# amcerbu/huygens

Hardware: AMD Instinct MI355X
Metric: band-samples/s (bands x frames/s) for 4096-band Filterbank (higher is better)
Workload: dtype f64; 1 GPU; C2 Filterbank<double>(order 2, 4096 bands), resonant band-pass f_i=0.5(i+1)SR/4096 R=0.999, boost 1 + open, k_p=0.1 k_g=1; samples_per_gpu=480000, bands=4096, bands_per_gpu=4096

## Files before the change

huygens_amd/_lib.py:

```python
from __future__ import annotations

import ctypes as C
import os
import re

_HERE = os.path.dirname(os.path.abspath(__file__))
LIB_PATH = os.environ.get("HZ_LIB_PATH") or os.path.join(_HERE, "lib", "libhuygens_hip.so")
HEADER_PATH = os.path.join(os.path.dirname(_HERE), "include", "huygens_hip.h")

HZ_OK = 0
HZ_E_INVALID = -1
HZ_E_RANGE = -2
HZ_E_HIP = -3
HZ_E_NODEV = -4
HZ_E_ALLOC = -5
HZ_E_UNSUPPORTED = -6
HZ_E_STATE = -7

HZ_FB_PATH_AUTO = 0
HZ_FB_PATH_GENERAL = 1
HZ_FB_PATH_LTI = 2
HZ_FB_PATH_RESPONSE = 3
HZ_FB_PATH_STREAM = 4

# ... 67 lines not shown
    "hz_fb_profile_read": (I, [VP, PD, PD, PD, C.POINTER(L)]),
    "hz_fb_set_target_groups": (I, [VP, I]),
    "hz_fb_set_path": (I, [VP, I]),
    "hz_fb_last_path": (I, [VP, C.POINTER(I)]),
    "hz_fb_tune_lti": (I, [VP, I, I, I]),
    "hz_fb_lti_plan": (I, [VP, C.POINTER(C.c_long), C.POINTER(C.c_long), C.POINTER(C.c_int)]),
    "hz_fb_lti_last_chunk": (I, [VP, C.POINTER(C.c_int)]),
    "hz_fb_set_response": (I, [VP, I]),
    "hz_fb_tune_response": (I, [VP, L, L]),
    "hz_fb_tune_response_engine": (I, [VP, I]),
    "hz_fb_sample_many": (I, [C.POINTER(VP), I, PD, I, D, PD]),
    "hz_fb_response_engine": (I, [VP, C.POINTER(I), C.POINTER(I)]),
    "hz_fb_tune_modal": (I, [VP, I]),
    "hz_fb_modal_info": (I, [VP, C.POINTER(I), C.POINTER(I), C.POINTER(I), C.POINTER(I)]),
    "hz_fb_response_info": (I, [VP, C.POINTER(L), C.POINTER(L), C.POINTER(I), C.POINTER(L)]),
    "hz_fb_get_response": (I, [VP, PD, L]),
    "hz_fb_set_bank_response": (I, [VP, PD, L]),
    "hz_fb_set_time_shard": (I, [VP, I, I]),
    "hz_fb_set_time_shard_fill": (I, [VP, I]),
    "hz_fb_time_shard_info": (I, [VP, C.POINTER(I), C.POINTER(L), C.POINTER(L), L]),
    "hz_fb_stationary_ready": (I, [VP, L, C.POINTER(I)]),
    "hz_fb_arm_time_shard": (I, [VP, I]),
    "hz_fb_tune_stream": (I, [VP, I]),
    "hz_fb_setter_seq": (I, [VP, C.POINTER(C.c_longlong)]),
    "hz_dly_sample": (I, [VP, VP, VP, I]),
    "hz_gran_sample": (I, [VP, D, PD]),
    "hz_rt_info": (I, [I, C.POINTER(C.c_longlong), C.POINTER(C.c_longlong), C.POINTER(I)]),
    "hz_add_lookahead_info": (I, [VP, C.POINTER(L), C.POINTER(L), C.POINTER(L)]),
    "hz_fb_stream_info": (I, [VP, C.POINTER(I), C.POINTER(L), C.POINTER(L), C.POINTER(I)]),
    "hz_osc_create": (I, [I, D, I, C.POINTER(VP)]),
# ... 202 lines not shown
```

huygens_amd/csrc/hz_fb_impl.h:

```cpp
#pragma once

#include <algorithm>
#include <atomic>
#include <chrono>
#include <cmath>
#include <cstring>
#include <mutex>
#include <optional>
#include <vector>

#include "hz_common.h"
#include "hz_fb_events.h"
#include "hz_mix.h"
#include "hz_mixplan.h"

namespace hz_fbi {

constexpr int kMaxOrder = 4;
constexpr int kLtiGeomChunk128 = 3;
constexpr int kStreamBlock = 1024;
constexpr size_t kLdsCeiling = 160 * 1024;

enum { MODE_MIX = 0, MODE_SEGEND = 1, MODE_STATE = 2 };

// ... 75 lines not shown
    std::vector<double> pg_host;
    long mirror_clock = 0;
    std::vector<long> mirror_at;
    bool converged = false;
    std::vector<hz::Event> sync_ev;
    hz::DevBuf<double> d_xhist_red;
    hz::PinBuf<double> tv_row;
    hz::Event tv_ev;
    bool tv_pending = false;
    int tv_kind = 0;
    double tv_param = 0;
    struct Resp {
        int mode = HZ_FB_RESP_EAGER;
        long K = -2;
        bool h_valid = false;
        long run = 0;
        bool implicit = false;
        long calls = 0;
        long min_call = 0;
        long bands_per_sample = -1;
        std::vector<double> h_over;
        bool over_valid = false;
        int shard_rank = 0, shard_world = 1;
        bool shard_zero = true;
        bool armed = false;
        hz::DevBuf<double> d_hist[2];
        int hcur = 0;
        hz::DevBuf<double> d_h;
        hz::DevBuf<double> d_hpart;
        hz::DevBuf<double> d_coef;
// ... 211 lines not shown
```

huygens_amd/csrc/hz_fb_mac.h:

```cpp
#pragma once

#include <hip/hip_runtime.h>

#include <algorithm>
#include <type_traits>

#include "hz_lds.h"

namespace hz_mac {

constexpr int kH = 2048;
constexpr int kMacR = 8;

enum StorePolicy { kStPlain = 0, kStThrough = 1 };
#ifndef HZ_ST_Y
#define HZ_ST_Y kStThrough
#endif
constexpr int kStY = HZ_ST_Y;
typedef unsigned int hz_u32x4 __attribute__((ext_vector_type(4)));
template <int POL>
struct Store16 {
    double2* base;
    __amdgpu_buffer_rsrc_t rs;
    __device__ __forceinline__ Store16(double2* b, unsigned bytes) : base(b) {
// ... 129 lines not shown
    const int b0 = (blockIdx.x / (kH / kMacBins)) * kMacBlk;
    HZ_DIAG_AT(1, 0);
    const long row_lo = (long)b0 + Q - QP;
    double2 hv[kHL], zv[kZL];
    auto hload = [&](auto k_) {
        constexpr int k = decltype(k_)::value;
        const double2 v = H[(long)(sl + 4 * k) * kH + q];
        hv[k] = make_double2(v.x, v.y);
    };
    auto zload = [&](auto k_) {
        constexpr int k = decltype(k_)::value;
        const int r = sl + 4 * k;
        const long row = row_lo + r;
        zv[k] = 4 * k + 3 < kZr || r < kZr ? Z[(row > 0 ? row : 0) * kH + q] : make_double2(0.0, 0.0);
    };
    constexpr int OS = S < QP ? S : (QP > 8 ? 8 : QP);
    static_for<0, QP / OS>([&](auto s_) {
        constexpr int s = decltype(s_)::value;
        static_for<s * OS / 4, (s + 1) * OS / 4>(hload);
        static_for_down<mac_zhi(QP, kZL, s, OS), mac_zlo(QP, s, OS)>(zload);
    });
    HZ_DIAG_VMCNT(kHL - OS / 4 + (QP - OS) / 4);
    HZ_DIAG_AT(1, 1);
    double ar[BPW], ai[BPW], zr[BPW], zi[BPW];
    static_for<0, NS>([&](auto s_) {
        constexpr int s = decltype(s_)::value;
        if constexpr (s == NS - 1) {
            HZ_DIAG_VMCNT(0);
            HZ_DIAG_AT(1, 2);
        }
        static_for<s * S / 4, (s + 1) * S / 4>([&](auto k_) {
// ... 43 lines not shown
            for (int r = 0; r < BPW; ++r) asm volatile("" : "+v"(ar[r]), "+v"(ai[r]));
            __builtin_amdgcn_sched_barrier(0);
        }
    });
    HZ_DIAG_AT(1, 3);
    const int nb = min(B - b0, kMacBlk);
    const Store16<kStY> yst(Y + (long)b0 * kH + q0, (unsigned)sizeof(double2) * ((nb - 1) * kH + kMacBins));
#pragma unroll
    for (int r = 0; r < BPW; ++r) {
        const int lb = BPW * sl + r;
        if (lb < nb) yst(lb * kH + lq, make_double2(ar[r], ai[r]));
    }
    HZ_DIAG_AT(1, 4);
}

constexpr int kMacChunk = 24;
constexpr int kMaccBins = 16;
constexpr size_t kMaccLdsBytes = sizeof(double2) * kMaccBins * (kMacChunk + (256 / kMaccBins) * kMacBpw + kMacChunk - 1);
__global__ __launch_bounds__(256) void resp_mac_kernel_ldsc(const double2* __restrict__ H, const double2* __restrict__ Z,
                                                            double2* __restrict__ Y, int Q, int B, int nch, int cps,
                                                            long ystride) {
    constexpr int BINS = kMaccBins, BPW = kMacBpw;
    constexpr int QP = kMacChunk, SL = 256 / BINS, kMacBlk = SL * BPW, kZr = kMacBlk + QP - 1;
    constexpr int kHL = (QP + SL - 1) / SL, kZL = (kZr + SL - 1) / SL;
    extern __shared__ double2 mac_lds[];
    double2(*hs)[BINS] = (double2(*)[BINS])mac_lds;
    double2(*zs)[BINS] = (double2(*)[BINS])(mac_lds + QP * BINS);
    const int t = threadIdx.x, lq = t & (BINS - 1), sl = t / BINS;
    const int q0 = (blockIdx.x % (kH / BINS)) * BINS, q = q0 + lq;
    const int b0 = (blockIdx.x / (kH / BINS)) * kMacBlk;
    double2 hv[kHL], zv[kZL];
// ... 68 lines not shown
template <int QP, int S = mac_stage<QP>()>
int launch_mac_lds_qp(int device, int B, const double2* H, const double2* Z, double2* Y, int Q, hipStream_t s) {
    if (int r = hz::allow_lds(device, (const void*)resp_mac_kernel_lds<QP, S>, mac_lds_bytes<QP>())) return r;
    hipLaunchKernelGGL((resp_mac_kernel_lds<QP, S>), dim3(mac_lds_grid(B)), dim3(256), (mac_lds_bytes<QP>()), s, H, Z, Y, Q, B);
    return HZ_OK;
}
inline int launch_mac_lds(int device, int Qp, int B, const double2* H, const double2* Z, double2* Y, int Q, hipStream_t s) {
    if (Qp > kMacChunk) {
        constexpr int blk = (256 / kMaccBins) * kMacBpw;
        const int ns = macc_splits(Qp), nch = Qp / kMacChunk, cps = (nch + ns - 1) / ns;
        const dim3 grid((unsigned)((kH / kMaccBins) * ((B + blk - 1) / blk)), (unsigned)ns);
        if (int r = hz::allow_lds(device, (const void*)resp_mac_kernel_ldsc, kMaccLdsBytes)) return r;
        hipLaunchKernelGGL(resp_mac_kernel_ldsc, grid, dim3(256), kMaccLdsBytes, s, H, Z, Y, Q, B, nch, cps, (long)B * kH);
        return HZ_OK;
    }
    if (Qp == 8) return launch_mac_lds_qp<8>(device, B, H, Z, Y, Q, s);
    if (Qp == 16) return launch_mac_lds_qp<16>(device, B, H, Z, Y, Q, s);
    return launch_mac_lds_qp<24>(device, B, H, Z, Y, Q, s);
}

typedef void (*MacKernel)(const double2*, const double2*, double2*, int, int, int);
inline MacKernel pick_mac(int Qp) {
    switch (Qp) {
    case 8: return resp_mac_kernel<kMacR, 8>;
    case 16: return resp_mac_kernel<kMacR, 16>;
    case 24: return resp_mac_kernel<kMacR, 24>;
    default: return resp_mac_kernel<kMacR, 0>;
    }
}

}
```

huygens_amd/csrc/hz_fb_resp.hip:

```cpp
#include <cstdio>
#include <cstdlib>
#include <cstdint>

#include "hz_fb_impl.h"
#include "hz_fb_state.h"
#include "hz_fft2k.h"
#include "hz_fb_col.h"
#include "hz_fb_modal.h"
#include "hz_fb_mac.h"

namespace {

constexpr int kLgP = 11, kP = 1 << kLgP;
constexpr int kF = 2 * kP;
constexpr int kLgH = kLgP, kH = kP;
constexpr int kThreads = 256;
constexpr int kPT = kH / kThreads;
constexpr long kMinCall = 16384;
constexpr long kBandsPerSample = 256;
static_assert(kH == hz2k::kN && kThreads == hz2k::kT, "hz_fft2k.h: 2048 points on 256 threads");

static_assert(kH == hz_mac::kH, "hz_fb_mac.h: the MAC's row length");

using hz_mac::kMacChunk;
// ... 147 lines not shown
    double2* Z;
    double* Zn;
    const double2* Y;
    int ys;
    long ystride;
    const double* Hn;
    double* out;
    double* hist_next;
    const double *pg, *pin, *gin;
    double* pg_next;
    double sp_n, sg_n;
    double* xhist_next;
    int N, O;
    int upkeep;
    int zero_outside;
};

__device__ __forceinline__ double resp_u(const RespArgs& a, long m) {
    m += a.off;
    if (m < a.K) return a.hist[m];
    m -= a.K;
    return m < a.off + a.n_out ? a.x[m] : 0.0;
}

struct WindowLoad {
    const RespArgs& a;
    long m0;
    __device__ __forceinline__ void operator()(double (&vr)[kPT], double (&vi)[kPT]) const {
        const int t = threadIdx.x;
        if (((a.K | a.off) & (kP - 1)) != 0) {
            const bool al = ((reinterpret_cast<uintptr_t>(a.hist) | reinterpret_cast<uintptr_t>(a.x)) & 15) == 0;
#pragma unroll
            for (int i = 0; i < kPT; ++i) {
                const int mm = 2 * (t + i * kThreads);
                const long m = m0 + mm + a.off;
                double2 v;
                if (al && m + 1 < a.K) v = *reinterpret_cast<const double2*>(a.hist + m);
                else if (al && m >= a.K && m + 1 - a.K < a.off + a.n_out) v = *reinterpret_cast<const double2*>(a.x + (m - a.K));
                else v = make_double2(resp_u(a, m0 + mm), resp_u(a, m0 + mm + 1));
                vr[i] = v.x;
                vi[i] = v.y;
            }
            return;
        }
        __amdgpu_buffer_rsrc_t rs[2];
#pragma unroll
        for (int h = 0; h < 2; ++h) {
            const long mh = m0 + a.off + h * kP;
            const long left = a.off + a.n_out - (mh - a.K);
            const double* bp = mh < a.K ? a.hist + mh : a.x + (mh - a.K);
            const int vl = mh < a.K ? kP : (int)(left <= 0 ? 0 : left >= kP ? kP : left);
            rs[h] = __builtin_amdgcn_make_buffer_rsrc(const_cast<double*>(bp), 0, 8 * vl, 0x00020000);
        }
#pragma unroll
        for (int i = 0; i < kPT; ++i) {
            const double2 v = __builtin_bit_cast(
                double2, __builtin_amdgcn_raw_buffer_load_b128(rs[i / 4], 16 * (t + (i & 3) * kThreads), 0, 0));
            vr[i] = v.x;
            vi[i] = v.y;
        }
    }
};

union RespLds {
    hz2k::Lds fft;
    hz_state::StateLds st;
    hz_modal::Lds2 md;
};
union RespFwdLds {
    hz2k::Lds fft;
    hz_modal::Lds1 m1;
    hz_modal::Lds2 m2;
};


__global__ __launch_bounds__(kThreads) void resp_fwd_kernel(RespArgs a, hz_modal::ModalArgs md) {
    __shared__ RespFwdLds u;
    if (md.on && (int)blockIdx.x >= a.nz) {
        HZ_DIAG_AT(0, 0);
        const int i = blockIdx.x - a.nz;
        if (i < md.n1) hz_modal::phase1_group(md, i, u.m1);
        else hz_modal::exc_partial(md, (i - md.n1) / md.exc_chunks, (i - md.n1) % md.exc_chunks, u.m2);
        HZ_DIAG_AT(0, 1);
        HZ_DIAG_AT(0, 2);
        HZ_DIAG_AT(0, 3);
        return;
    }
    real_window_fwd<kStZ>(u.fft, WindowLoad{a, (long)blockIdx.x * kP}, a.twf, a.Z + (long)blockIdx.x * kH,
                          a.Zn + blockIdx.x, true);
}

typedef void (*RespKernel)(RespArgs, hz_state::StateArgs, hz_modal::ModalArgs);
// ... 178 lines not shown
    if (i >= K) return;
    const long m = n + i;
    hist_next[i] = m < K ? hist[m] : x[m - K];
}

typedef void (*RespHKernel)(const double*, const double*, const double*, const double*, int, long, double*);
RespHKernel pick_h(int O) {
    switch (O) {
    case 1: return resp_h_kernel<1>;
    case 2: return resp_h_kernel<2>;
    case 3: return resp_h_kernel<3>;
    default: return resp_h_kernel<4>;
    }
}

int q_padded(int Q) { return Q > 24 ? (Q + 23) / 24 * 24 : (Q + kMacR - 1) / kMacR * kMacR; }

bool col_q_ok(int Q) { return Q == 8 || Q == 16 || Q == 24; }
typedef void (*ColKernel)(hz_col::ColArgs);
ColKernel pick_col(int Q) {
    return Q == 8 ? resp_col_kernel<8> : Q == 16 ? resp_col_kernel<16> : resp_col_kernel<24>;
}

int resp_setup(hz_fb* h) {
    hz_fb::Resp& R = h->resp;
    if (R.K == -2) {
        R.K = hz_fbi::fb_horizon(h, -53);
        if (R.K >= 0) R.K = std::max<long>(8192, (R.K + 8191) / 8192 * 8192);
        R.h_valid = false;
        R.run = 0;
    }
// ... 38 lines not shown
        }
        HZ_TRY(R.d_tw.reserve(2 * tab.size()));
        HZ_TRY_HIP(hipMemcpy(R.d_tw, tab.data(), sizeof(double2) * tab.size(), hipMemcpyHostToDevice));
    }
    return HZ_OK;
}

int modal_prepare(hz_fb* h);

int resp_build_h(hz_fb* h) {
    hz_fb::Resp& R = h->resp;
    if (R.h_valid) return HZ_OK;
    const int O = h->order, N = h->N;
    const long K = R.K;
    const int G = (N + 63) / 64;
    const int Q = (int)(K / kP), Qp = q_padded(Q);
    HZ_TRY(R.d_coef.reserve((size_t)N * (2 * O + 1)));
    HZ_TRY_HIP(hipMemcpyAsync(R.d_coef, h->F.data(), sizeof(double) * N * (O + 1), hipMemcpyHostToDevice, h->stream));
    HZ_TRY_HIP(hipMemcpyAsync(R.d_coef + (size_t)N * (O + 1), h->B.data(), sizeof(double) * N * O,
                              hipMemcpyHostToDevice, h->stream));
    HZ_TRY(R.d_hpart.reserve((size_t)G * K));
    HZ_TRY(R.d_h.reserve((size_t)K));
    HZ_TRY(R.d_H.reserve((size_t)Qp * (2 * kH + 1)));
    HZ_TRY_HIP(hipMemsetAsync(R.d_H, 0, sizeof(double) * (size_t)Qp * (2 * kH + 1), h->stream));
    hipLaunchKernelGGL(pick_h(O), dim3(G), dim3(64), 0, h->stream, (const double*)R.d_coef,
                       (const double*)(R.d_coef + (size_t)N * (O + 1)), (const double*)h->d_pin,
                       (const double*)h->d_gin, N, K, R.d_hpart);
    HZ_TRY_HIP(hipGetLastError());
    hipLaunchKernelGGL(resp_hsum_kernel, dim3((unsigned)((K + 255) / 256)), dim3(256), 0, h->stream,
                       (const double*)R.d_hpart, G, K, R.d_h);
    HZ_TRY_HIP(hipGetLastError());
    if (R.over_valid)
        HZ_TRY_HIP(hipMemcpyAsync(R.d_h, R.h_over.data(), sizeof(double) * K, hipMemcpyHostToDevice, h->stream));
    hipLaunchKernelGGL(resp_hspec_kernel, dim3((unsigned)Q), dim3(kThreads), 0, h->stream, (const double*)R.d_h, K,
                       (const double2*)R.d_tw.get() + kTwFwd, (double2*)R.d_H.get(), R.d_H + (size_t)Qp * 2 * kH);
    HZ_TRY_HIP(hipGetLastError());
    if (col_q_ok(Q)) {
        HZ_TRY(R.d_Hc.reserve((size_t)hz_col::kSlots * Q * 64 * 2));
        hipLaunchKernelGGL(hz_col::resp_hcol_kernel, dim3(hz_col::kSlots, (unsigned)Q), dim3(64), 0, h->stream,
                           (const double2*)R.d_H.get(), (const double*)(R.d_H + (size_t)Qp * 2 * kH), Q, (double2*)R.d_Hc.get());
        HZ_TRY_HIP(hipGetLastError());
    }
    HZ_TRY(hz_fbi::fb_state_prepare(h));
    HZ_TRY(modal_prepare(h));
    HZ_TRY_HIP(hipStreamSynchronize(h->stream));
    R.h_valid = true;
    ++R.h_gen;
    return HZ_OK;
}

int resp_states(hz_fb* h, double* ystate) {
    hz_fb::Resp& R = h->resp;
    return hz_fbi::fb_state_window(h, R.d_hist[R.hcur], R.K, ystate, h->stream);
}

int modal_prepare(hz_fb* h) {
    using namespace hz_modal;
// ... 208 lines not shown
    HZ_TRY(resp_setup(h));
    hipLaunchKernelGGL(resp_hist_kernel, dim3((unsigned)((R.K + 255) / 256)), dim3(256), 0, h->stream,
                       (const double*)R.d_hist[R.hcur], d_in, R.K, n, R.d_hist[R.hcur ^ 1]);
    HZ_TRY_HIP(hipGetLastError());
    R.hcur ^= 1;
    R.run = std::min(R.run + n, 1L << 60);
    return HZ_OK;
}

int fb_launch_resp(hz_fb* h, const double* d_in, double* d_out, long n) {
    hz_fb::Resp& R = h->resp;
    HZ_TRY(resp_setup(h));
    HZ_TRY(fb_stream_to_hist(h));
    HZ_TRY(resp_build_h(h));
    const long K = R.K;
    const int Q = (int)(K / kP), Qp = q_padded(Q);
    long off = 0, n_out = n;
    if (R.shard_world > 1 && R.over_valid) {
        const long Ball = (n + kP - 1) / kP;
        const long lo = Ball * R.shard_rank / R.shard_world, hi = Ball * (R.shard_rank + 1) / R.shard_world;
        off = std::min(n, lo * kP);
        n_out = std::min(n, hi * kP) - off;
    }
    const int B = (int)std::max<long>(1, (n_out + kP - 1) / kP);
    const int nz = Q + B - 1;
    const int zrows = (B + 128 - 1) / 128 * 128 + Qp;
    if ((size_t)zrows * (2 * kH + 1) > R.d_Z.cap()) {
        HZ_TRY(R.d_Z.reserve((size_t)zrows * (2 * kH + 1)));
        HZ_TRY_HIP(hipMemsetAsync(R.d_Z, 0, sizeof(double) * R.d_Z.cap(), h->stream));
    }
    const size_t zn_at = (size_t)zrows * 2 * kH;
    const int ys = Qp > kMacChunk ? macc_splits(Qp) : 1;
    HZ_TRY(R.d_Y.reserve((size_t)ys * B * kH * 2));
    hipEvent_t* e = nullptr;
    if (h->prof) {
        HZ_TRY(fb_prof_events(h, &e));
        HZ_TRY_HIP(hipEventRecord(e[0], h->stream));
        h->ev_skip[h->ev.index_of(e) / 5] |= 2;
    }
    RespArgs a;
    a.hist = R.d_hist[R.hcur];
    a.x = d_in;
    a.K = K;
    a.n = n;
    a.off = off;
    a.n_out = n_out;
    a.Q = Q;
    a.B = B;
    a.twf = (const double2*)R.d_tw.get() + kTwFwd;
    a.twi = (const double2*)R.d_tw.get() + kTwInv;
    a.Z = (double2*)R.d_Z.get();
    a.Zn = R.d_Z + zn_at;
    a.Y = (const double2*)R.d_Y.get();
    a.ys = ys;
    a.ystride = (long)B * kH;
    a.Hn = R.d_H + (size_t)Qp * 2 * kH;
    a.out = d_out;
    a.hist_next = R.d_hist[R.hcur ^ 1];
    a.pg = h->d_pg[h->scur];
    a.pg_next = h->d_pg[h->scur ^ 1];
    a.pin = h->d_pin;
    a.gin = h->d_gin;
    a.sp_n = (double)powl((long double)h->sp, (long double)n);
    a.sg_n = (double)powl((long double)h->sg, (long double)n);
    a.xhist_next = h->d_xhist[h->xcur ^ 1];
    a.N = h->N;
    a.O = h->order;
    a.nz = nz;
    a.upkeep = 1;
    a.zero_outside = R.shard_zero ? 1 : 0;
    const bool lazy = R.mode == HZ_FB_RESP_LAZY;
    const bool col = R.col_on && col_q_ok(Q);
    const bool modal = !lazy && n >= 3 && R.modal_on && R.modal_ok && !col;
    const bool chained = !lazy && n >= K && h->order <= 2 && !modal;
    const bool inside = chained || modal;
    hz_state::StateArgs st = hz_state::StateArgs();
    if (chained) HZ_TRY(fb_state_chained(h, d_in + (n - K), K, h->d_ystate[h->scur ^ 1], &st));
    hz_modal::ModalArgs md = hz_modal::ModalArgs();
    if (modal) modal_args(h, R.d_hist[R.hcur], d_in, n, h->d_ystate[h->scur ^ 1], &md);
    const int so = chained ? h->order : 0;
    const int nm1 = modal ? md.n1 + md.nexc * md.exc_chunks : 0;
    const int nm2 = modal ? md.n2p + (md.nexc ? 1 : 0) : 0;
    md.first2 = B;
    md.n2 = nm2;
    R.last_engine = col ? 1 : modal ? 2 : 0;
    R.modal_last = modal;
    if (col) {
// ... 74 lines not shown
        static long long hv[3][1024][hz_mac::kDiagStamps];
        if (hipMemcpyFromSymbol(hv, HIP_SYMBOL(hz_mac::g_diag), sizeof(hv)) == hipSuccess) {
            const int nmac = Qp <= kMacChunk ? (int)hz_mac::mac_lds_grid(B) : 0;
            const int tot[3] = {std::min((int)nz + nm1, 1024), std::min(nmac, 1024), std::min((int)B + nm2, 1024)};
            if (nmac > 0) {
                long long t0 = hv[1][0][0];
                for (int i = 0; i < tot[1]; ++i) t0 = std::min(t0, hv[1][i][0]);
                double ph[4] = {0, 0, 0, 0}, smax = 0, emax = 0;
                for (int i = 0; i < tot[1]; ++i) {
                    smax = std::max(smax, (hv[1][i][0] - t0) * 0.01);
                    emax = std::max(emax, (hv[1][i][4] - t0) * 0.01);
                    for (int j = 0; j < 4; ++j) ph[j] += (hv[1][i][j + 1] - hv[1][i][j]) * 0.01;
                }
                std::fprintf(stderr, "[mac stamps] %d workgroups (B = %d, Qp = %d, stages of %d steps): mean first stage "
                             "landed %.2f us, all landed + %.2f us, MAC steps done + %.2f us, stores %.2f us; starts up "
                             "to %.2f us, last end %.2f us\n", tot[1], B, Qp, Qp == 16 ? hz_mac::mac_stage<16>() :
                             Qp == 24 ? hz_mac::mac_stage<24>() : Qp, ph[0] / tot[1], ph[1] / tot[1], ph[2] / tot[1],
                             ph[3] / tot[1], smax, emax);
            }
            for (int k = 0; k < 3; k += 2) {
                long long t0 = hv[k][0][0];
                for (int i = 0; i < tot[k]; ++i) t0 = std::min(t0, hv[k][i][0]);
                double ph[3] = {0, 0, 0}, emain = 0, eextra = 0, smax = 0;
                int nmain = 0, nextra = 0;
                for (int i = 0; i < tot[k]; ++i) {
                    const bool extra = k == 0 ? i >= nz : k == 2 ? i >= B : false;
                    const double e = (hv[k][i][3] - t0) * 0.01;
                    smax = std::max(smax, (hv[k][i][0] - t0) * 0.01);
                    if (extra) {
                        ++nextra;
                        eextra = std::max(eextra, e);
                    } else {
                        ++nmain;
                        emain = std::max(emain, e);
                        for (int j = 0; j < 3; ++j) ph[j] += (hv[k][i][j + 1] - hv[k][i][j]) * 0.01;
                    }
                }
                if (k == 0) {
                    static const char* const kClass[5] = {"history windows", "straddling window", "call windows",
                                                          "phase-1 workgroups", "exceptional partials"};
                    struct {
                        int cnt = 0;
                        double first = 1e30, last = 0, ph[3] = {0, 0, 0};
                    } c[5];
                    for (int i = 0; i < tot[0]; ++i) {
                        const long m = off + (long)i * kP;
                        const int cl = i >= nz ? (i < nz + md.n1 ? 3 : 4) : m + kF <= K ? 0 : m < K ? 1 : 2;
                        ++c[cl].cnt;
                        c[cl].first = std::min(c[cl].first, (hv[0][i][0] - t0) * 0.01);
                        c[cl].last = std::max(c[cl].last, (hv[0][i][3] - t0) * 0.01);
                        for (int j = 0; j < 3; ++j) c[cl].ph[j] += (hv[0][i][j + 1] - hv[0][i][j]) * 0.01;
                    }
                    for (int cl = 0; cl < 5; ++cl)
                        if (c[cl].cnt)
                            std::fprintf(stderr, "[fwd stamps] %-20s %4d: first start %.2f us, mean operands %.2f us, compute %.2f us, "
                                         "stores %.2f us, last end %.2f us\n", kClass[cl], c[cl].cnt, c[cl].first,
                                         c[cl].ph[0] / c[cl].cnt, c[cl].ph[1] / c[cl].cnt, c[cl].ph[2] / c[cl].cnt, c[cl].last);
                }
                std::fprintf(stderr, "[%s stamps] %d workgroups: mean operands %.2f us, compute %.2f us, stores %.2f us; "
                             "starts up to %.2f us, last end %.2f us; %d modal workgroups, last end %.2f us\n",
                             k == 0 ? "fwd" : k == 1 ? "mac" : "inv", nmain, ph[0] / std::max(nmain, 1),
                             ph[1] / std::max(nmain, 1), ph[2] / std::max(nmain, 1), smax, emain, nextra, eextra);
            }
        }
    }
#endif
    if (e && inside) HZ_TRY_HIP(hipEventRecord(e[4], h->stream));
    if (e && !inside) HZ_TRY_HIP(hipEventRecord(e[2], h->stream));
    R.hcur ^= 1;
    R.run = std::min(R.run + n, 1L << 60);
    if (lazy) {
        R.implicit = true;
// ... 5 lines not shown
        if (e) HZ_TRY_HIP(hipEventRecord(e[3], h->stream));
        HZ_TRY(resp_states(h, h->d_ystate[h->scur ^ 1]));
        if (e) HZ_TRY_HIP(hipEventRecord(e[4], h->stream));
        R.implicit = false;
    }
    h->prof_launches += h->prof ? 1 : 0;
    ++R.calls;
    fb_advance(h, n);
    return HZ_OK;
}

int fb_resp_tail_spectra(hz_fb* h, long K1) {
    hz_fb::Resp& R = h->resp;
    hz_fb::Resp::Stream& S = R.st;
    const long Kt = R.K - K1;
    const int Q = (int)(Kt / kP), Qp = q_padded(Q);
    HZ_TRY(S.d_tH.reserve((size_t)Qp * (2 * kH + 1)));
    HZ_TRY_HIP(hipMemsetAsync(S.d_tH, 0, sizeof(double) * (size_t)Qp * (2 * kH + 1), h->stream));
    hipLaunchKernelGGL(resp_hspec_kernel, dim3((unsigned)Q), dim3(kThreads), 0, h->stream, (const double*)(R.d_h + K1),
                       Kt, (const double2*)R.d_tw.get() + kTwFwd, (double2*)S.d_tH.get(), S.d_tH + (size_t)Qp * 2 * kH);
    HZ_TRY_HIP(hipGetLastError());
    S.tQ = Q;
    return HZ_OK;
}

int fb_resp_tail_conv(hz_fb* h, const double* u, long n, double* out, hipStream_t st) {
    hz_fb::Resp& R = h->resp;
    hz_fb::Resp::Stream& S = R.st;
    const int Q = S.tQ, Qp = q_padded(Q);
    const long Kt = (long)Q * kP;
    const int B = (int)((n + kP - 1) / kP), nz = Q + B - 1;
    const int zrows = (B + 64 - 1) / 64 * 64 + Qp;
    if ((size_t)zrows * (2 * kH + 1) > S.d_tZ.cap()) {
        HZ_TRY(S.d_tZ.reserve((size_t)zrows * (2 * kH + 1)));
        HZ_TRY_HIP(hipMemsetAsync(S.d_tZ, 0, sizeof(double) * S.d_tZ.cap(), st));
    }
    HZ_TRY(S.d_tY.reserve((size_t)B * kH * 2));
    RespArgs a{};
    a.hist = u;
    a.x = u + Kt;
    a.K = Kt;
    a.n = n;
    a.off = 0;
    a.n_out = n;
    a.Q = Q;
    a.B = B;
    a.nz = nz;
    a.twf = (const double2*)R.d_tw.get() + kTwFwd;
    a.twi = (const double2*)R.d_tw.get() + kTwInv;
    a.Z = (double2*)S.d_tZ.get();
    a.Zn = S.d_tZ + (size_t)zrows * 2 * kH;
    a.Y = (const double2*)S.d_tY.get();
    a.ys = 1;
    a.Hn = S.d_tH + (size_t)Qp * 2 * kH;
    a.out = out;
    a.upkeep = 0;
// ... 1 lines not shown
    hipLaunchKernelGGL(resp_fwd_kernel, dim3((unsigned)nz), dim3(kThreads), 0, st, a, hz_modal::ModalArgs());
    HZ_TRY_HIP(hipGetLastError());
    const int nmac = (kH / 256) * ((B + kMacR - 1) / kMacR);
    hipLaunchKernelGGL(pick_mac(Qp), dim3((unsigned)nmac), dim3(256), 0, st, (const double2*)S.d_tH.get(),
                       (const double2*)S.d_tZ.get(), (double2*)S.d_tY.get(), Q, Qp, B);
    HZ_TRY_HIP(hipGetLastError());
    hipLaunchKernelGGL(resp_inv_kernel<0>, dim3((unsigned)B), dim3(kThreads), 0, st, a, hz_state::StateArgs(),
                       hz_modal::ModalArgs());
    HZ_TRY_HIP(hipGetLastError());
    return HZ_OK;
}

void fb_resp_free(hz_fb* h) {
    hz_fb::Resp& R = h->resp;
    fb_stream_free(h);
    const bool col_on = R.col_on, modal_on = R.modal_on;
    R = hz_fb::Resp();
    R.col_on = col_on;
    R.modal_on = modal_on;
}

}

extern "C" {

int hz_fb_set_response(hz_fb* h, int mode) {
    if (!h || mode < HZ_FB_RESP_OFF || mode > HZ_FB_RESP_LAZY) {
        hz::set_error("hz_fb_set_response: mode must be HZ_FB_RESP_OFF, _EAGER or _LAZY");
        return HZ_E_INVALID;
    }
    hz_fbi::Entry entry(h, "hz_fb_set_response");
    HZ_TRY(entry.status);
    HZ_TRY(hz_fbi::fb_resp_materialize(h));
    h->resp.mode = mode;
// ... 115 lines not shown
    if (active) *active = on ? 1 : 0;
    if (first) *first = lo;
    if (count) *count = cnt;
    return HZ_OK;
}

int hz_fb_response_info(hz_fb* h, long* horizon, long* run, int* implicit_state, long* calls) {
    if (!h) return HZ_E_INVALID;
    if (horizon) *horizon = h->resp.K;
    if (run) *run = h->resp.run;
    if (implicit_state) *implicit_state = h->resp.implicit ? 1 : 0;
    if (calls) *calls = h->resp.calls;
    return HZ_OK;
}

int hz_fb_get_response(hz_fb* h, double* out, long count) {
    if (!h || !out || count < 0) return HZ_E_INVALID;
    hz_fbi::Entry entry(h, "hz_fb_get_response", false);
    HZ_TRY(entry.status);
    HZ_TRY(hz_fbi::fb_upload(h));
    if (h->order == 0) {
        hz::set_error("hz_fb_get_response: order 0 bank");
        return HZ_E_INVALID;
    }
    HZ_TRY(resp_setup(h));
    if (h->resp.K <= 0) {
        hz::set_error("hz_fb_get_response: no finite horizon (some band needs more than 2^18 samples)");
        return HZ_E_UNSUPPORTED;
    }
    HZ_TRY(resp_build_h(h));
// ... 9 lines not shown
```

huygens_amd/filterbank.py:

```python
from __future__ import annotations

import ctypes as C

import numpy as np

from ._lib import HZ_DIST_NONE, HZ_DIST_SOFTCLIP, PD, check, dptr, load


TV_COEFFS, TV_RESONANT = 0, 1
EV_BOOST, EV_MIX = 0, 1

FB_EVENT = np.dtype([("at", np.int64), ("band", np.int32), ("kind", np.int32), ("value", np.float64)])


def pack_events(events) -> np.ndarray:
    if isinstance(events, np.ndarray) and events.dtype == FB_EVENT:
        return np.ascontiguousarray(events)
    if isinstance(events, tuple) and len(events) == 4 and all(np.ndim(e) == 1 for e in events):
        cols = [np.asarray(e) for e in events]
        if len({len(c) for c in cols}) != 1:
            raise ValueError("process_events: the four event arrays differ in length")
    else:
        ev = list(events or ())
        cols = [np.asarray([e[i] for e in ev]) for i in range(4)]
# ... 188 lines not shown
        return bool(a.value), b.value == 1

    def tune_modal(self, on: bool = True):
        check(self._lib.hz_fb_tune_modal(self._h, 1 if on else 0))

    def modal_info(self):
        v = [C.c_int() for _ in range(4)]
        check(self._lib.hz_fb_modal_info(self._h, *[C.byref(x) for x in v]))
        return bool(v[0].value), bool(v[1].value), v[2].value, bool(v[3].value)

    def response_info(self):
        k, r, i, c = C.c_long(), C.c_long(), C.c_int(), C.c_long()
        check(self._lib.hz_fb_response_info(self._h, C.byref(k), C.byref(r), C.byref(i), C.byref(c)))
        return k.value, r.value, bool(i.value), c.value

    def response(self, count: int) -> np.ndarray:
        out = np.zeros(count)
        check(self._lib.hz_fb_get_response(self._h, dptr(out), count))
        return out

    def set_bank_response(self, h):
        v = np.ascontiguousarray(h, dtype=np.float64)
        check(self._lib.hz_fb_set_bank_response(self._h, dptr(v), len(v)))

    def set_time_shard(self, rank: int, world: int):
        check(self._lib.hz_fb_set_time_shard(self._h, int(rank), int(world)))

    def set_time_shard_fill(self, zero_outside: bool = True):
        check(self._lib.hz_fb_set_time_shard_fill(self._h, 1 if zero_outside else 0))

# ... 38 lines not shown
```

include/huygens_hip.h:

```cpp
#ifndef HUYGENS_HIP_H
#define HUYGENS_HIP_H

#include <stddef.h>

#ifdef __cplusplus
extern "C" {
#endif

#define HZ_OK 0
#define HZ_E_INVALID (-1)
#define HZ_E_RANGE (-2)
#define HZ_E_HIP (-3)
#define HZ_E_NODEV (-4)
#define HZ_E_ALLOC (-5)
#define HZ_E_UNSUPPORTED (-6)
#define HZ_E_STATE (-7)

#define HZ_DIST_NONE 0
#define HZ_DIST_SOFTCLIP 1
#define HZ_DIST_SATURATE 2
#define HZ_DIST_LIMITER 3
#define HZ_SOFTCLIP_WIDTH 0.125
#define HZ_DIST_DEFAULT_PARAM(dist_id) ((dist_id) == HZ_DIST_SOFTCLIP ? HZ_SOFTCLIP_WIDTH : 0.0)

// ... 38 lines not shown
#define HZ_FB_PATH_LTI 2
#define HZ_FB_PATH_RESPONSE 3
#define HZ_FB_PATH_STREAM 4
int hz_fb_set_path(hz_fb* h, int path);
int hz_fb_last_path(hz_fb* h, int* path);
#define HZ_FB_RESP_OFF 0
#define HZ_FB_RESP_EAGER 1
#define HZ_FB_RESP_LAZY 2
int hz_fb_set_response(hz_fb* h, int mode);
int hz_fb_tune_response(hz_fb* h, long min_call, long bands_per_sample);
int hz_fb_tune_response_engine(hz_fb* h, int column_split);
int hz_fb_response_engine(hz_fb* h, int* column_split_on, int* last_call_column_split);
int hz_fb_tune_modal(hz_fb* h, int on);
int hz_fb_modal_info(hz_fb* h, int* on, int* qualifies, int* exceptional, int* last_call);
int hz_fb_response_info(hz_fb* h, long* horizon, long* run, int* implicit_state, long* calls);
int hz_fb_get_response(hz_fb* h, double* out, long count);
int hz_fb_set_bank_response(hz_fb* h, const double* resp, long count);
int hz_fb_set_time_shard(hz_fb* h, int rank, int world);
int hz_fb_set_time_shard_fill(hz_fb* h, int zero_outside);
int hz_fb_stationary_ready(hz_fb* h, long n, int* ready);
int hz_fb_arm_time_shard(hz_fb* h, int armed);
int hz_fb_time_shard_info(hz_fb* h, int* active, long* first, long* count, long n);
int hz_fb_tune_stream(hz_fb* h, int enable);
int hz_fb_stream_info(hz_fb* h, int* enabled, long* block, long* calls, int* history_in_ring);
int hz_fb_tune_lti(hz_fb* h, int chunk, int bands_per_wave, int waves_per_group);
int hz_fb_lti_plan(hz_fb* h, long* nseg, long* skip_tiles, int* fine_parts);
int hz_fb_lti_last_chunk(hz_fb* h, int* chunk);

int hz_rt_info(int device, long long* requests, long long* launches, int* active);

// ... 261 lines not shown
```

Before: 89640 billion band-samples/s.

## Truncate response convolution to partitions above double-precision tail bound

Adds an opt-in tuning switch that scans the bank's impulse response on the host and drops trailing convolution partitions whose remaining L1 mass is below 2^-53 of the total. The history pointer and tap count passed to the forward and MAC kernels are shifted so only the truncated length is convolved. Padding now rounds to multiples of 4 instead of 8, with new MAC kernel instantiations for 4, 12 and 20 partitions. The switch is off by default, so the default path only changes through the finer padding and a reordered spectrum build.

New measurement: 88110 billion band-samples/s. 1.7% lower.

```diff
diff --git a/huygens_amd/_lib.py b/huygens_amd/_lib.py
--- a/huygens_amd/_lib.py
+++ b/huygens_amd/_lib.py
@@ -105,6 +105,8 @@
     "hz_fb_tune_modal": (I, [VP, I]),
     "hz_fb_modal_info": (I, [VP, C.POINTER(I), C.POINTER(I), C.POINTER(I), C.POINTER(I)]),
     "hz_fb_response_info": (I, [VP, C.POINTER(L), C.POINTER(L), C.POINTER(I), C.POINTER(L)]),
+    "hz_fb_response_conv_info": (I, [VP, C.POINTER(I), C.POINTER(L), PD]),
+    "hz_fb_tune_conv_horizon": (I, [VP, I]),
     "hz_fb_get_response": (I, [VP, PD, L]),
     "hz_fb_set_bank_response": (I, [VP, PD, L]),
     "hz_fb_set_time_shard": (I, [VP, I, I]),
diff --git a/huygens_amd/csrc/hz_fb_impl.h b/huygens_amd/csrc/hz_fb_impl.h
--- a/huygens_amd/csrc/hz_fb_impl.h
+++ b/huygens_amd/csrc/hz_fb_impl.h
@@ -113,6 +113,9 @@
         int mode = HZ_FB_RESP_EAGER;
         long K = -2;
         bool h_valid = false;
+        bool conv_tune = false;
+        int Qc = 0;
+        double conv_tail = 0.0;
         long run = 0;
         bool implicit = false;
         long calls = 0;
diff --git a/huygens_amd/csrc/hz_fb_mac.h b/huygens_amd/csrc/hz_fb_mac.h
--- a/huygens_amd/csrc/hz_fb_mac.h
+++ b/huygens_amd/csrc/hz_fb_mac.h
@@ -5,6 +5,7 @@
 #include <algorithm>
 #include <type_traits>
 
+#include "hz_fb_qpad.h"
 #include "hz_lds.h"
 
 namespace hz_mac {
@@ -167,7 +168,7 @@
         const long row = row_lo + r;
         zv[k] = 4 * k + 3 < kZr || r < kZr ? Z[(row > 0 ? row : 0) * kH + q] : make_double2(0.0, 0.0);
     };
-    constexpr int OS = S < QP ? S : (QP > 8 ? 8 : QP);
+    constexpr int OS = S < QP ? S : (QP <= 8 ? QP : QP % 8 == 0 ? 8 : 4);
     static_for<0, QP / OS>([&](auto s_) {
         constexpr int s = decltype(s_)::value;
         static_for<s * OS / 4, (s + 1) * OS / 4>(hload);
@@ -241,7 +242,6 @@
     HZ_DIAG_AT(1, 4);
 }
 
-constexpr int kMacChunk = 24;
 constexpr int kMaccBins = 16;
 constexpr size_t kMaccLdsBytes = sizeof(double2) * kMaccBins * (kMacChunk + (256 / kMaccBins) * kMacBpw + kMacChunk - 1);
 __global__ __launch_bounds__(256) void resp_mac_kernel_ldsc(const double2* __restrict__ H, const double2* __restrict__ Z,
@@ -340,16 +340,25 @@
         hipLaunchKernelGGL(resp_mac_kernel_ldsc, grid, dim3(256), kMaccLdsBytes, s, H, Z, Y, Q, B, nch, cps, (long)B * kH);
         return HZ_OK;
     }
-    if (Qp == 8) return launch_mac_lds_qp<8>(device, B, H, Z, Y, Q, s);
-    if (Qp == 16) return launch_mac_lds_qp<16>(device, B, H, Z, Y, Q, s);
-    return launch_mac_lds_qp<24>(device, B, H, Z, Y, Q, s);
+    switch (Qp) {
+    case 4: return launch_mac_lds_qp<4>(device, B, H, Z, Y, Q, s);
+    case 8: return launch_mac_lds_qp<8>(device, B, H, Z, Y, Q, s);
+    case 12: return launch_mac_lds_qp<12>(device, B, H, Z, Y, Q, s);
+    case 16: return launch_mac_lds_qp<16>(device, B, H, Z, Y, Q, s);
+    case 20: return launch_mac_lds_qp<20>(device, B, H, Z, Y, Q, s);
+    case 24: return launch_mac_lds_qp<24>(device, B, H, Z, Y, Q, s);
+    default: hz::set_error("launch_mac_lds: %d partitions (a multiple of 4 up to 24, or chunks of 24)", Qp); return HZ_E_INVALID;
+    }
 }
 
 typedef void (*MacKernel)(const double2*, const double2*, double2*, int, int, int);
 inline MacKernel pick_mac(int Qp) {
     switch (Qp) {
+    case 4: return resp_mac_kernel<kMacR, 4>;
     case 8: return resp_mac_kernel<kMacR, 8>;
+    case 12: return resp_mac_kernel<kMacR, 12>;
     case 16: return resp_mac_kernel<kMacR, 16>;
+    case 20: return resp_mac_kernel<kMacR, 20>;
     case 24: return resp_mac_kernel<kMacR, 24>;
     default: return resp_mac_kernel<kMacR, 0>;
     }
diff --git a/huygens_amd/csrc/hz_fb_qpad.h b/huygens_amd/csrc/hz_fb_qpad.h
--- /dev/null
+++ b/huygens_amd/csrc/hz_fb_qpad.h
@@ -0,0 +1,9 @@
+#pragma once
+
+namespace hz_mac {
+
+constexpr int kMacChunk = 24;
+
+constexpr int mac_q_padded(int Q) { return Q > kMacChunk ? (Q + kMacChunk - 1) / kMacChunk * kMacChunk : (Q + 3) / 4 * 4; }
+
+}
diff --git a/huygens_amd/csrc/hz_fb_resp.hip b/huygens_amd/csrc/hz_fb_resp.hip
--- a/huygens_amd/csrc/hz_fb_resp.hip
+++ b/huygens_amd/csrc/hz_fb_resp.hip
@@ -1,6 +1,8 @@
+#include <cmath>
 #include <cstdio>
 #include <cstdlib>
 #include <cstdint>
+#include <vector>
 
 #include "hz_fb_impl.h"
 #include "hz_fb_state.h"
@@ -185,12 +187,14 @@
     int N, O;
     int upkeep;
     int zero_outside;
+    const double* chist;
+    long Kc;
 };
 
 __device__ __forceinline__ double resp_u(const RespArgs& a, long m) {
     m += a.off;
-    if (m < a.K) return a.hist[m];
-    m -= a.K;
+    if (m < a.Kc) return a.chist[m];
+    m -= a.Kc;
     return m < a.off + a.n_out ? a.x[m] : 0.0;
 }
 
@@ -199,15 +203,15 @@
     long m0;
     __device__ __forceinline__ void operator()(double (&vr)[kPT], double (&vi)[kPT]) const {
         const int t = threadIdx.x;
-        if (((a.K | a.off) & (kP - 1)) != 0) {
-            const bool al = ((reinterpret_cast<uintptr_t>(a.hist) | reinterpret_cast<uintptr_t>(a.x)) & 15) == 0;
+        if (((a.Kc | a.off) & (kP - 1)) != 0) {
+            const bool al = ((reinterpret_cast<uintptr_t>(a.chist) | reinterpret_cast<uintptr_t>(a.x)) & 15) == 0;
 #pragma unroll
             for (int i = 0; i < kPT; ++i) {
                 const int mm = 2 * (t + i * kThreads);
                 const long m = m0 + mm + a.off;
                 double2 v;
-                if (al && m + 1 < a.K) v = *reinterpret_cast<const double2*>(a.hist + m);
-                else if (al && m >= a.K && m + 1 - a.K < a.off + a.n_out) v = *reinterpret_cast<const double2*>(a.x + (m - a.K));
+                if (al && m + 1 < a.Kc) v = *reinterpret_cast<const double2*>(a.chist + m);
+                else if (al && m >= a.Kc && m + 1 - a.Kc < a.off + a.n_out) v = *reinterpret_cast<const double2*>(a.x + (m - a.Kc));
                 else v = make_double2(resp_u(a, m0 + mm), resp_u(a, m0 + mm + 1));
                 vr[i] = v.x;
                 vi[i] = v.y;
@@ -218,9 +222,9 @@
 #pragma unroll
         for (int h = 0; h < 2; ++h) {
             const long mh = m0 + a.off + h * kP;
-            const long left = a.off + a.n_out - (mh - a.K);
-            const double* bp = mh < a.K ? a.hist + mh : a.x + (mh - a.K);
-            const int vl = mh < a.K ? kP : (int)(left <= 0 ? 0 : left >= kP ? kP : left);
+            const long left = a.off + a.n_out - (mh - a.Kc);
+            const double* bp = mh < a.Kc ? a.chist + mh : a.x + (mh - a.Kc);
+            const int vl = mh < a.Kc ? kP : (int)(left <= 0 ? 0 : left >= kP ? kP : left);
             rs[h] = __builtin_amdgcn_make_buffer_rsrc(const_cast<double*>(bp), 0, 8 * vl, 0x00020000);
         }
 #pragma unroll
@@ -247,6 +251,11 @@
 
 __global__ __launch_bounds__(kThreads) void resp_fwd_kernel(RespArgs a, hz_modal::ModalArgs md) {
     __shared__ RespFwdLds u;
+#ifdef HZ_DIAG_STAMPS
+    if (threadIdx.x == 0 && blockIdx.x < 1024)
+        hz_mac::g_diag[0][blockIdx.x][4] = ((long long)__builtin_amdgcn_s_getreg((31 << 11) | 20) << 32) |
+                                           (unsigned)__builtin_amdgcn_s_getreg((31 << 11) | 4);
+#endif
     if (md.on && (int)blockIdx.x >= a.nz) {
         HZ_DIAG_AT(0, 0);
         const int i = blockIdx.x - a.nz;
@@ -455,7 +464,23 @@
     }
 }
 
-int q_padded(int Q) { return Q > 24 ? (Q + 23) / 24 * 24 : (Q + kMacR - 1) / kMacR * kMacR; }
+int q_padded(int Q) { return hz_mac::mac_q_padded(Q); }
+int q_padded_tail(int Q) { return Q > 24 ? (Q + 23) / 24 * 24 : (Q + kMacR - 1) / kMacR * kMacR; }
+
+int resp_conv_horizon(const double* hh, long K, double* tail) {
+    const int Q = (int)(K / kP);
+    std::vector<double> at((size_t)Q + 1, 0.0);
+    double acc = 0.0;
+    for (long t = K - 1; t >= 0; --t) {
+        acc += std::fabs(hh[t]);
+        if (t % kP == 0) at[(size_t)(t / kP)] = acc;
+    }
+    const double bound = std::ldexp(at[0], -53);
+    int qc = Q;
+    while (qc > 1 && at[(size_t)qc - 1] <= bound) --qc;
+    *tail = at[0] > 0.0 ? at[(size_t)qc] / at[0] : 0.0;
+    return qc;
+}
 
 bool col_q_ok(int Q) { return Q == 8 || Q == 16 || Q == 24; }
 typedef void (*ColKernel)(hz_col::ColArgs);
@@ -524,15 +549,14 @@
     const int O = h->order, N = h->N;
     const long K = R.K;
     const int G = (N + 63) / 64;
-    const int Q = (int)(K / kP), Qp = q_padded(Q);
+    const int Q = (int)(K / kP);
     HZ_TRY(R.d_coef.reserve((size_t)N * (2 * O + 1)));
     HZ_TRY_HIP(hipMemcpyAsync(R.d_coef, h->F.data(), sizeof(double) * N * (O + 1), hipMemcpyHostToDevice, h->stream));
     HZ_TRY_HIP(hipMemcpyAsync(R.d_coef + (size_t)N * (O + 1), h->B.data(), sizeof(double) * N * O,
                               hipMemcpyHostToDevice, h->stream));
     HZ_TRY(R.d_hpart.reserve((size_t)G * K));
     HZ_TRY(R.d_h.reserve((size_t)K));
-    HZ_TRY(R.d_H.reserve((size_t)Qp * (2 * kH + 1)));
-    HZ_TRY_HIP(hipMemsetAsync(R.d_H, 0, sizeof(double) * (size_t)Qp * (2 * kH + 1), h->stream));
+    HZ_TRY(R.d_H.reserve((size_t)std::max(Q, q_padded(Q)) * (2 * kH + 1)));
     hipLaunchKernelGGL(pick_h(O), dim3(G), dim3(64), 0, h->stream, (const double*)R.d_coef,
                        (const double*)(R.d_coef + (size_t)N * (O + 1)), (const double*)h->d_pin,
                        (const double*)h->d_gin, N, K, R.d_hpart);
@@ -542,15 +566,28 @@
     HZ_TRY_HIP(hipGetLastError());
     if (R.over_valid)
         HZ_TRY_HIP(hipMemcpyAsync(R.d_h, R.h_over.data(), sizeof(double) * K, hipMemcpyHostToDevice, h->stream));
-    hipLaunchKernelGGL(resp_hspec_kernel, dim3((unsigned)Q), dim3(kThreads), 0, h->stream, (const double*)R.d_h, K,
+    R.Qc = Q;
+    R.conv_tail = 0.0;
+    if (R.conv_tune) {
+        std::vector<double> hh((size_t)K);
+        HZ_TRY_HIP(hipMemcpyAsync(hh.data(), R.d_h, sizeof(double) * K, hipMemcpyDeviceToHost, h->stream));
+        HZ_TRY_HIP(hipStreamSynchronize(h->stream));
+        R.Qc = resp_conv_horizon(hh.data(), K, &R.conv_tail);
+    }
+    if (col_q_ok(Q)) {
+        hipLaunchKernelGGL(resp_hspec_kernel, dim3((unsigned)Q), dim3(kThreads), 0, h->stream, (const double*)R.d_h, K,
+                           (const double2*)R.d_tw.get() + kTwFwd, (double2*)R.d_H.get(), R.d_H + (size_t)Q * 2 * kH);
+        HZ_TRY_HIP(hipGetLastError());
+        HZ_TRY(R.d_Hc.reserve((size_t)hz_col::kSlots * Q * 64 * 2));
+        hipLaunchKernelGGL(hz_col::resp_hcol_kernel, dim3(hz_col::kSlots, (unsigned)Q), dim3(64), 0, h->stream,
+                           (const double2*)R.d_H.get(), (const double*)(R.d_H + (size_t)Q * 2 * kH), Q, (double2*)R.d_Hc.get());
+        HZ_TRY_HIP(hipGetLastError());
+    }
+    const int Qc = R.Qc, Qp = q_padded(Qc);
+    HZ_TRY_HIP(hipMemsetAsync(R.d_H, 0, sizeof(double) * (size_t)Qp * (2 * kH + 1), h->stream));
+    hipLaunchKernelGGL(resp_hspec_kernel, dim3((unsigned)Qc), dim3(kThreads), 0, h->stream, (const double*)R.d_h, K,
                        (const double2*)R.d_tw.get() + kTwFwd, (double2*)R.d_H.get(), R.d_H + (size_t)Qp * 2 * kH);
     HZ_TRY_HIP(hipGetLastError());
-    if (col_q_ok(Q)) {
-        HZ_TRY(R.d_Hc.reserve((size_t)hz_col::kSlots * Q * 64 * 2));
-        hipLaunchKernelGGL(hz_col::resp_hcol_kernel, dim3(hz_col::kSlots, (unsigned)Q), dim3(64), 0, h->stream,
-                           (const double2*)R.d_H.get(), (const double*)(R.d_H + (size_t)Qp * 2 * kH), Q, (double2*)R.d_Hc.get());
-        HZ_TRY_HIP(hipGetLastError());
-    }
     HZ_TRY(hz_fbi::fb_state_prepare(h));
     HZ_TRY(modal_prepare(h));
     HZ_TRY_HIP(hipStreamSynchronize(h->stream));
@@ -789,7 +826,9 @@
     HZ_TRY(fb_stream_to_hist(h));
     HZ_TRY(resp_build_h(h));
     const long K = R.K;
-    const int Q = (int)(K / kP), Qp = q_padded(Q);
+    const bool col = R.col_on && col_q_ok((int)(K / kP));
+    const int Q = col ? (int)(K / kP) : R.Qc, Qp = q_padded(Q);
+    const long Kc = (long)Q * kP;
     long off = 0, n_out = n;
     if (R.shard_world > 1 && R.over_valid) {
         const long Ball = (n + kP - 1) / kP;
@@ -817,6 +856,8 @@
     a.hist = R.d_hist[R.hcur];
     a.x = d_in;
     a.K = K;
+    a.chist = a.hist + (K - Kc);
+    a.Kc = Kc;
     a.n = n;
     a.off = off;
     a.n_out = n_out;
@@ -845,7 +886,6 @@
     a.upkeep = 1;
     a.zero_outside = R.shard_zero ? 1 : 0;
     const bool lazy = R.mode == HZ_FB_RESP_LAZY;
-    const bool col = R.col_on && col_q_ok(Q);
     const bool modal = !lazy && n >= 3 && R.modal_on && R.modal_ok && !col;
     const bool chained = !lazy && n >= K && h->order <= 2 && !modal;
     const bool inside = chained || modal;
@@ -950,8 +990,8 @@
                 }
                 std::fprintf(stderr, "[mac stamps] %d workgroups (B = %d, Qp = %d, stages of %d steps): mean first stage "
                              "landed %.2f us, all landed + %.2f us, MAC steps done + %.2f us, stores %.2f us; starts up "
-                             "to %.2f us, last end %.2f us\n", tot[1], B, Qp, Qp == 16 ? hz_mac::mac_stage<16>() :
-                             Qp == 24 ? hz_mac::mac_stage<24>() : Qp, ph[0] / tot[1], ph[1] / tot[1], ph[2] / tot[1],
+                             "to %.2f us, last end %.2f us\n", tot[1], B, Qp, hz_mac::mac_stage_of(Qp, HZ_MAC_STAGE),
+                             ph[0] / tot[1], ph[1] / tot[1], ph[2] / tot[1],
                              ph[3] / tot[1], smax, emax);
             }
             for (int k = 0; k < 3; k += 2) {
@@ -981,7 +1021,7 @@
                     } c[5];
                     for (int i = 0; i < tot[0]; ++i) {
                         const long m = off + (long)i * kP;
-                        const int cl = i >= nz ? (i < nz + md.n1 ? 3 : 4) : m + kF <= K ? 0 : m < K ? 1 : 2;
+                        const int cl = i >= nz ? (i < nz + md.n1 ? 3 : 4) : m + kF <= Kc ? 0 : m < Kc ? 1 : 2;
                         ++c[cl].cnt;
                         c[cl].first = std::min(c[cl].first, (hv[0][i][0] - t0) * 0.01);
                         c[cl].last = std::max(c[cl].last, (hv[0][i][3] - t0) * 0.01);
@@ -992,6 +1032,62 @@
                             std::fprintf(stderr, "[fwd stamps] %-20s %4d: first start %.2f us, mean operands %.2f us, compute %.2f us, "
                                          "stores %.2f us, last end %.2f us\n", kClass[cl], c[cl].cnt, c[cl].first,
                                          c[cl].ph[0] / c[cl].cnt, c[cl].ph[1] / c[cl].cnt, c[cl].ph[2] / c[cl].cnt, c[cl].last);
+                    const int nw = std::min((int)nz, 1024);
+                    auto cu_of = [&](int i) {
+                        const long long w = hv[0][i][4];
+                        return (int)((((w >> 32) & 15) << 8) | (((w >> 13) & 7) << 5) | (((w >> 12) & 1) << 4) | ((w >> 8) & 15));
+                    };
+                    std::vector<int> per(16 << 8, 0);
+                    for (int i = 0; i < nw; ++i) ++per[cu_of(i)];
+                    int cus = 0, ncrowd = 0;
+                    double alone = 0, crowd = 0;
+                    for (int cnt : per) cus += cnt > 0;
+                    for (int i = 0; i < nw; ++i) {
+                        const double e = (hv[0][i][3] - t0) * 0.01;
+                        if (per[cu_of(i)] > 1) {
+                            ++ncrowd;
+                            crowd = std::max(crowd, e);
+                        } else {
+                            alone = std::max(alone, e);
+                        }
+                    }
+                    std::fprintf(stderr, "[fwd windows] %d windows on %d CUs: %d alone on theirs, last end %.2f us; %d shared a CU, "
+                                 "last end %.2f us\n", nw, cus, nw - ncrowd, alone, ncrowd, crowd);
+                    for (int i = std::max(0, nw - 6); i < nw; ++i)
+                        std::fprintf(stderr, "[fwd windows] blockIdx %3d: start %.2f us, end %.2f us, XCC %d SE %d SH %d CU %2d, %d "
+                                     "windows on that CU\n", i, (hv[0][i][0] - t0) * 0.01, (hv[0][i][3] - t0) * 0.01, cu_of(i) >> 8,
+                                     (cu_of(i) >> 5) & 7, (cu_of(i) >> 4) & 1, cu_of(i) & 15, per[cu_of(i)]);
+                    std::vector<int> pm(16 << 8, 0);
+                    for (int i = nw; i < tot[0]; ++i) ++pm[cu_of(i)];
+                    int nmod = 0;
+                    double e_mod = 0, e_free = 0, s_mod = 0, s_free = 0;
+                    std::vector<int> order(nw);
+                    for (int i = 0; i < nw; ++i) {
+                        order[i] = i;
+                        const double e = (hv[0][i][3] - t0) * 0.01;
+                        if (pm[cu_of(i)] > 0) {
+                            ++nmod;
+                            e_mod = std::max(e_mod, e);
+                            s_mod += e;
+                        } else {
+                            e_free = std::max(e_free, e);
+                            s_free += e;
+                        }
+                    }
+                    std::fprintf(stderr, "[fwd windows] %d windows with a modal workgroup on their CU: mean end %.2f us, last %.2f us; "
+                                 "%d without: mean end %.2f us, last %.2f us\n", nmod, s_mod / std::max(nmod, 1), e_mod, nw - nmod,
+                                 s_free / std::max(nw - nmod, 1), e_free);
+                    std::sort(order.begin(), order.end(), [&](int x, int y) { return hv[0][x][3] > hv[0][y][3]; });
+                    for (int j = 0; j < std::min(nw, 6); ++j) {
+                        const int i = order[j];
+                        std::fprintf(stderr, "[fwd windows] ended last: blockIdx %3d, end %.2f us, %d windows and %d modal workgroups on "
+                                     "its CU\n", i, (hv[0][i][3] - t0) * 0.01, per[cu_of(i)], pm[cu_of(i)]);
+                    }
+                    for (int i = 0; i < nw; ++i)
+                        if (per[cu_of(i)] > 1 && i < nw - 6)
+                            std::fprintf(stderr, "[fwd windows] blockIdx %3d shared: start %.2f us, end %.2f us, XCC %d SE %d SH %d "
+                                         "CU %2d\n", i, (hv[0][i][0] - t0) * 0.01, (hv[0][i][3] - t0) * 0.01, cu_of(i) >> 8,
+                                         (cu_of(i) >> 5) & 7, (cu_of(i) >> 4) & 1, cu_of(i) & 15);
                 }
                 std::fprintf(stderr, "[%s stamps] %d workgroups: mean operands %.2f us, compute %.2f us, stores %.2f us; "
                              "starts up to %.2f us, last end %.2f us; %d modal workgroups, last end %.2f us\n",
@@ -1027,7 +1123,7 @@
     hz_fb::Resp& R = h->resp;
     hz_fb::Resp::Stream& S = R.st;
     const long Kt = R.K - K1;
-    const int Q = (int)(Kt / kP), Qp = q_padded(Q);
+    const int Q = (int)(Kt / kP), Qp = q_padded_tail(Q);
     HZ_TRY(S.d_tH.reserve((size_t)Qp * (2 * kH + 1)));
     HZ_TRY_HIP(hipMemsetAsync(S.d_tH, 0, sizeof(double) * (size_t)Qp * (2 * kH + 1), h->stream));
     hipLaunchKernelGGL(resp_hspec_kernel, dim3((unsigned)Q), dim3(kThreads), 0, h->stream, (const double*)(R.d_h + K1),
@@ -1040,7 +1136,7 @@
 int fb_resp_tail_conv(hz_fb* h, const double* u, long n, double* out, hipStream_t st) {
     hz_fb::Resp& R = h->resp;
     hz_fb::Resp::Stream& S = R.st;
-    const int Q = S.tQ, Qp = q_padded(Q);
+    const int Q = S.tQ, Qp = q_padded_tail(Q);
     const long Kt = (long)Q * kP;
     const int B = (int)((n + kP - 1) / kP), nz = Q + B - 1;
     const int zrows = (B + 64 - 1) / 64 * 64 + Qp;
@@ -1053,6 +1149,8 @@
     a.hist = u;
     a.x = u + Kt;
     a.K = Kt;
+    a.chist = u;
+    a.Kc = Kt;
     a.n = n;
     a.off = 0;
     a.n_out = n;
@@ -1084,10 +1182,11 @@
 void fb_resp_free(hz_fb* h) {
     hz_fb::Resp& R = h->resp;
     fb_stream_free(h);
-    const bool col_on = R.col_on, modal_on = R.modal_on;
+    const bool col_on = R.col_on, modal_on = R.modal_on, conv_tune = R.conv_tune;
     R = hz_fb::Resp();
     R.col_on = col_on;
     R.modal_on = modal_on;
+    R.conv_tune = conv_tune;
 }
 
 }
@@ -1233,6 +1332,34 @@
     return HZ_OK;
 }
 
+int hz_fb_response_conv_info(hz_fb* h, int* partitions, long* taps, double* tail_over_l1) {
+    hz_fbi::Entry entry(h, "hz_fb_response_conv_info", false);
+    HZ_TRY(entry.status);
+    HZ_TRY(hz_fbi::fb_upload(h));
+    if (h->order == 0) {
+        hz::set_error("hz_fb_response_conv_info: order 0 bank");
+        return HZ_E_INVALID;
+    }
+    HZ_TRY(resp_setup(h));
+    if (h->resp.K <= 0) {
+        hz::set_error("hz_fb_response_conv_info: no finite horizon (some band needs more than 2^18 samples)");
+        return HZ_E_UNSUPPORTED;
+    }
+    HZ_TRY(resp_build_h(h));
+    if (partitions) *partitions = h->resp.Qc;
+    if (taps) *taps = (long)h->resp.Qc * kP;
+    if (tail_over_l1) *tail_over_l1 = h->resp.conv_tail;
+    return HZ_OK;
+}
+
+int hz_fb_tune_conv_horizon(hz_fb* h, int on) {
+    if (!h) return HZ_E_INVALID;
+    hz_fbi::HandleLock lk(h);
+    if (h->resp.conv_tune != (on != 0)) h->resp.h_valid = false;
+    h->resp.conv_tune = on != 0;
+    return HZ_OK;
+}
+
 int hz_fb_get_response(hz_fb* h, double* out, long count) {
     if (!h || !out || count < 0) return HZ_E_INVALID;
     hz_fbi::Entry entry(h, "hz_fb_get_response", false);
diff --git a/huygens_amd/filterbank.py b/huygens_amd/filterbank.py
--- a/huygens_amd/filterbank.py
+++ b/huygens_amd/filterbank.py
@@ -226,6 +226,14 @@
         check(self._lib.hz_fb_response_info(self._h, C.byref(k), C.byref(r), C.byref(i), C.byref(c)))
         return k.value, r.value, bool(i.value), c.value
 
+    def response_conv_info(self):
+        q, t, r = C.c_int(), C.c_long(), C.c_double()
+        check(self._lib.hz_fb_response_conv_info(self._h, C.byref(q), C.byref(t), C.byref(r)))
+        return q.value, t.value, r.value
+
+    def tune_conv_horizon(self, on: bool = True):
+        check(self._lib.hz_fb_tune_conv_horizon(self._h, 1 if on else 0))
+
     def response(self, count: int) -> np.ndarray:
         out = np.zeros(count)
         check(self._lib.hz_fb_get_response(self._h, dptr(out), count))
diff --git a/include/huygens_hip.h b/include/huygens_hip.h
--- a/include/huygens_hip.h
+++ b/include/huygens_hip.h
@@ -76,6 +76,8 @@
 int hz_fb_tune_modal(hz_fb* h, int on);
 int hz_fb_modal_info(hz_fb* h, int* on, int* qualifies, int* exceptional, int* last_call);
 int hz_fb_response_info(hz_fb* h, long* horizon, long* run, int* implicit_state, long* calls);
+int hz_fb_tune_conv_horizon(hz_fb* h, int on);
+int hz_fb_response_conv_info(hz_fb* h, int* partitions, long* taps, double* tail_over_l1);
 int hz_fb_get_response(hz_fb* h, double* out, long count);
 int hz_fb_set_bank_response(hz_fb* h, const double* resp, long count);
 int hz_fb_set_time_shard(hz_fb* h, int rank, int world);
```
